# hyperconnect/TC-ResNet

Measured on AMD Instinct MI355X. Metric: utterances/sec (1 s@16 kHz) TCResNet8-1.0 forward, higher is better.
Workload: dtype f32; 1 GPU; TCResNet8-1.0 eval forward, waveform->softmax, batch 4096/GPU, 49x40 MFCC (40/20 ms, FFT 1024), 12 classes; global_batch=4096, parallelism=dp1 (utterance shards, no collective)

## Files before the change

include/tcresnet_hip.h:

```cpp
#ifndef TCRESNET_HIP_H
#define TCRESNET_HIP_H

#include <stddef.h>
#include <stdint.h>

#ifdef __cplusplus
extern "C" {
#endif

#define TCR_ABI_VERSION 3
#define TCR_HALO 4
#define TCR_MAX_BLOCKS 16

typedef enum tcr_status {
    TCR_OK = 0,
    TCR_ERR_ARG = -1,
    TCR_ERR_HIP = -2,
    TCR_ERR_WORKSPACE = -3
} tcr_status;

int tcr_abi_version(void);
const char* tcr_last_error(void);
static inline int tcr_padded_len(int t) { return t + 2 * TCR_HALO; }

// ... 230 lines not shown
                    float* logits, float* probs, float* smoothed, int32_t* top, float* score, int32_t* is_new, void* stream);

#define TCR_FAMILY_TCRESNET 0
#define TCR_FAMILY_DSCNN 1
#define TCR_FAMILY_G2D 2
typedef struct tcr_model_ref {
    int family;
    const void* handle;
    const float* params;
    const float* aux;
} tcr_model_ref;

size_t tcr_stream_state_bytes_m(const tcr_frontend_cfg* cfg, const tcr_model_ref* model, int n_streams, int k, const tcr_detect_cfg* det);
size_t tcr_stream_workspace_bytes_m(const tcr_frontend_cfg* cfg, const tcr_model_ref* model, int n_streams, int k);
int tcr_stream_init_m(const tcr_frontend_cfg* cfg, const void* plan_dev, const tcr_model_ref* model, int n_streams, int k,
                      const tcr_detect_cfg* det, void* state, void* workspace, size_t ws_bytes, void* stream);
int tcr_stream_step_m(const tcr_frontend_cfg* cfg, const void* plan_dev, const tcr_model_ref* model, int n_streams, int k,
                      const tcr_detect_cfg* det, const float* samples, const uint8_t* reset, void* state, void* workspace,
                      size_t ws_bytes, float* logits, float* probs, float* smoothed, int32_t* top, float* score, int32_t* is_new,
                      void* stream);
size_t tcr_scan_workspace_bytes_m(const tcr_frontend_cfg* cfg, const tcr_model_ref* model, int k, int max_windows);
int tcr_scan_m(const tcr_frontend_cfg* cfg, const void* plan_dev, const tcr_model_ref* model, int n_signals, int64_t n_samples, int k,
               const tcr_detect_cfg* det, const float* samples, void* workspace, size_t ws_bytes, float* logits, float* probs,
               float* smoothed, int32_t* top, float* score, int32_t* is_new, void* stream);
int tcr_stream_scan_m(const tcr_frontend_cfg* cfg, const void* plan_dev, const tcr_model_ref* model, int n_streams, int64_t n_samples,
                      int k, const tcr_detect_cfg* det, const float* samples, const uint8_t* reset, void* state, void* workspace,
                      size_t ws_bytes, float* logits, float* probs, float* smoothed, int32_t* top, float* score, int32_t* is_new,
                      void* stream);

int tcr_detect_sweep(int n_signals, int64_t steps, int num_classes, const int32_t* top, const float* score,
                     const int64_t* valid_steps, int32_t suppression_steps, int n_thresholds, const float* thresholds,
                     const int32_t* event_offsets, const int64_t* event_first, const int64_t* event_last,
                     const int32_t* event_label, int32_t* detections, int32_t* hits, int32_t* duplicates,
                     uint8_t* fired, void* stream);

typedef struct {
    int32_t up, down, taps;
    int32_t in_format;
    int32_t in_step;
} tcr_resample_cfg;
int tcr_resample(const tcr_resample_cfg* cfg, const float* table, int n_streams, const void* in, int64_t in_pitch, int64_t in_first,
                 int64_t n_in, int64_t out_first, int64_t n_out, float* out, int64_t out_pitch, void* stream);
int tcr_resample_span(const tcr_resample_cfg* cfg, int64_t out_first, int64_t n_out, int64_t* first, int64_t* n);

const char* tcr_kernel_name(int index);

enum { TCR_TUNE_CONV_PATH = 0,
       TCR_TUNE_FRONTEND = 1,
       TCR_TUNE_CONV_B = 2,
       TCR_TUNE_NET_FUSED = 3,
       TCR_TUNE_FUSED_GROUP = 4,
       TCR_TUNE_FUSED_WAVES = 5,
       TCR_TUNE_CONV_KSPLIT = 6,
       TCR_TUNE_WGRAD_STREAM = 7,
       TCR_TUNE_TRAIN_FWD = 8,
       TCR_TUNE_TRAIN_BWD = 9,
       TCR_TUNE_PHASE_CFG = 10,
       TCR_TUNE_BWD_BN_FUSED = 11,
       TCR_TUNE_BWD_MASK = 12,
       TCR_TUNE_FE_GRID = 13,
       TCR_TUNE_FUSED_GRID = 14,
       TCR_TUNE_DS_TRAIN = 15,
       TCR_TUNE_WGRAD_TILES = 16,
       TCR_TUNE_DOWN_DGRAD = 17,
       TCR_TUNE_BWD_LAZY_CFG = 18,
       TCR_TUNE_PHASE_STATIC = 19,
       TCR_TUNE_WGRAD_WAVES = 20,
       TCR_TUNE_WGRAD_LDS = 21,
       TCR_TUNE_LAZY_STAGE = 22,
       TCR_TUNE_FE_KERNEL = 23,
       TCR_TUNE_FE_STAGGER = 24,
       TCR_TUNE_PW_WGRAD = 25,
       TCR_TUNE_DEPLOY_F32 = 26,
       TCR_TUNE_NET_SMALL = 27,
       TCR_TUNE_PW_POS = 28,
       TCR_TUNE_BN_APPLY = 29,
       TCR_TUNE_DW_DGRAD = 30,
       TCR_TUNE_DW_WGRAD = 31,
       TCR_TUNE_DW_FWD = 32,
       TCR_TUNE_WGRAD_PIPE = 33,
       TCR_TUNE_COUNT = 34 };
int tcr_tune(int knob, int value);

void* tcr_internal_stream(int idx, void* caller_stream);

#ifdef __cplusplus
}
#endif
#endif
```

tc-resnet_amd/_lib.py:

```python
from __future__ import annotations

import ctypes as C
import os
from typing import Optional

HALO = 4
MAX_BLOCKS = 16
ABI_VERSION = 3
_HERE = os.path.dirname(os.path.abspath(__file__))
HIP_LIB_PATH = os.path.join(_HERE, "lib", "libtcresnet_hip.so")


class TcrError(RuntimeError):
    pass


class FrontendCfg(C.Structure):
    _fields_ = [("sample_rate", C.c_int32), ("n_samples", C.c_int32), ("win", C.c_int32), ("hop", C.c_int32),
                ("nfft", C.c_int32), ("n_frames", C.c_int32), ("n_mel", C.c_int32), ("n_coef", C.c_int32),
                ("lower_hz", C.c_float), ("upper_hz", C.c_float), ("method", C.c_int32)]


class TCResNetCfg(C.Structure):
    _fields_ = [("scope", C.c_char * 32), ("in_channels", C.c_int32), ("t_in", C.c_int32), ("num_classes", C.c_int32),
                ("n_blocks", C.c_int32), ("channels", C.c_int32 * (MAX_BLOCKS + 1)), ("bn_decay", C.c_float),
                ("bn_eps", C.c_float)]


class DSCNNCfg(C.Structure):
    _fields_ = [("h_in", C.c_int32), ("w_in", C.c_int32), ("num_classes", C.c_int32), ("depth", C.c_int32),
                ("n_separable", C.c_int32), ("conv1_kh", C.c_int32), ("conv1_kw", C.c_int32), ("conv1_sh", C.c_int32),
                ("conv1_sw", C.c_int32), ("ds1_sh", C.c_int32), ("ds1_sw", C.c_int32), ("bn_decay", C.c_float),
                ("bn_eps", C.c_float)]


class DetectCfg(C.Structure):
    _fields_ = [("average_steps", C.c_int32), ("min_count", C.c_int32), ("suppression_steps", C.c_int32), ("threshold", C.c_float)]


class ResampleCfg(C.Structure):
    _fields_ = [("up", C.c_int32), ("down", C.c_int32), ("taps", C.c_int32), ("in_format", C.c_int32), ("in_step", C.c_int32)]


FAMILY_TCRESNET, FAMILY_DSCNN, FAMILY_G2D = 0, 1, 2


class ModelRef(C.Structure):
    _fields_ = [("family", C.c_int), ("handle", C.c_void_p), ("params", C.c_void_p), ("aux", C.c_void_p)]


class TensorInfo(C.Structure):
    _fields_ = [("name", C.c_char * 96), ("kind", C.c_int32), ("arena", C.c_int32), ("offset", C.c_int64),
                ("size", C.c_int64), ("shape", C.c_int32 * 4), ("rank", C.c_int32)]


_P = C.c_void_p
_PROTOTYPES = {
    "tcr_abi_version": (C.c_int, []),
    "tcr_last_error": (C.c_char_p, []),
    "tcr_kernel_name": (C.c_char_p, [C.c_int]),
    "tcr_tune": (C.c_int, [C.c_int, C.c_int]),
    "tcr_internal_stream": (_P, [C.c_int, _P]),
    "tcr_frontend_resolve": (C.c_int, [C.POINTER(FrontendCfg)]),
    "tcr_frontend_plan_bytes": (C.c_size_t, [C.POINTER(FrontendCfg)]),
    "tcr_frontend_plan_init": (C.c_int, [C.POINTER(FrontendCfg), _P]),
    "tcr_frontend_plan_mel_matrix": (C.c_int, [C.POINTER(FrontendCfg), _P, _P]),
    "tcr_frontend_plan_dct_matrix": (C.c_int, [C.POINTER(FrontendCfg), _P, _P]),
    "tcr_frontend_fwd": (C.c_int, [C.POINTER(FrontendCfg), _P, _P, C.c_int, _P, _P]),
    "tcr_frontend_fwd_rounds": (C.c_int, [C.POINTER(FrontendCfg), _P, _P, C.c_int, _P, C.c_int, _P]),
    "tcr_features_to_planar": (C.c_int, [_P, C.c_int, C.c_int, C.c_int, _P, _P]),
    "tcr_features_from_planar": (C.c_int, [_P, C.c_int, C.c_int, C.c_int, _P, _P]),
    "tcr_tcresnet_create": (C.c_int, [C.POINTER(TCResNetCfg), C.POINTER(_P)]),
    "tcr_net_destroy": (None, [_P]),
    "tcr_net_param_floats": (C.c_int64, [_P]),
    "tcr_net_decay_floats": (C.c_int64, [_P]),
    "tcr_net_stat_floats": (C.c_int64, [_P]),
    "tcr_net_num_tensors": (C.c_int, [_P]),
    "tcr_net_tensor_info": (C.c_int, [_P, C.c_int, C.POINTER(TensorInfo)]),
    "tcr_net_out_frames": (C.c_int, [_P]),
    "tcr_net_feat_channels": (C.c_int, [_P]),
    "tcr_net_workspace_bytes": (C.c_size_t, [_P, C.c_int, C.c_int]),
    "tcr_net_forward_infer": (C.c_int, [_P, _P, _P, _P, C.c_int, _P, C.c_size_t, _P, _P, _P, _P]),
    "tcr_net_forward_train": (C.c_int, [_P, _P, _P, _P, _P, C.c_int, C.c_int, C.c_float, C.c_uint64, C.c_int64,
                                        C.c_float, _P, C.c_size_t, _P, _P, _P, _P]),
    "tcr_net_frozen_floats": (C.c_int64, [_P]),
    "tcr_net_fold_bn": (C.c_int, [_P, _P, _P, _P, _P]),
    "tcr_net_forward_frozen": (C.c_int, [_P, _P, _P, _P, C.c_int, _P, C.c_size_t, _P, _P, _P, _P]),
    "tcr_forward_waveform": (C.c_int, [C.POINTER(FrontendCfg), _P, _P, _P, _P, _P, C.c_int, _P, C.c_int, _P, _P, C.c_size_t, _P, _P, _P, _P]),
    "tcr_net_backward": (C.c_int, [_P, _P, _P, C.c_int, _P, C.c_size_t, _P, _P]),
    "tcr_net_num_stages": (C.c_int, [_P, C.c_int]),
    "tcr_net_stage_sums": (C.c_int, [_P, C.c_int, C.c_int, _P, C.c_int, C.POINTER(_P), C.POINTER(C.c_int64)]),
    "tcr_net_forward_train_stage": (C.c_int, [_P, _P, _P, _P, _P, C.c_int, C.c_int, C.c_float, C.c_uint64, C.c_int64,
                                              C.c_float, _P, C.c_size_t, _P, _P, _P, C.c_int, _P]),
    "tcr_net_backward_stage": (C.c_int, [_P, _P, _P, C.c_int, C.c_int, _P, C.c_size_t, _P, C.c_int, _P]),
    "tcr_net_num_levels": (C.c_int, [_P, C.c_int]),
    "tcr_net_level_sums": (C.c_int, [_P, C.c_int, C.c_int, _P, C.c_int, C.POINTER(_P), C.POINTER(C.c_int64)]),
    "tcr_net_forward_train_level": (C.c_int, [_P, _P, _P, _P, _P, C.c_int, C.c_int, C.c_float, C.c_uint64, C.c_int64,
                                              C.c_float, _P, C.c_size_t, _P, _P, _P, C.c_int, _P]),
    "tcr_net_backward_level": (C.c_int, [_P, _P, _P, C.c_int, C.c_int, _P, C.c_size_t, _P, C.c_int, _P]),
    "tcr_dscnn_create": (C.c_int, [C.POINTER(DSCNNCfg), C.POINTER(_P)]),
    "tcr_dscnn_destroy": (None, [_P]),
    "tcr_dscnn_param_floats": (C.c_int64, [_P]),
    "tcr_dscnn_stat_floats": (C.c_int64, [_P]),
    "tcr_dscnn_num_tensors": (C.c_int, [_P]),
    "tcr_dscnn_tensor_info": (C.c_int, [_P, C.c_int, C.POINTER(TensorInfo)]),
    "tcr_dscnn_workspace_bytes": (C.c_size_t, [_P, C.c_int]),
    "tcr_dscnn_forward_infer": (C.c_int, [_P, _P, _P, _P, C.c_int, _P, C.c_size_t, _P, _P, _P]),
    "tcr_augment_fwd": (C.c_int, [_P, _P, _P, _P, _P, _P, _P, C.c_int, C.c_int, _P, _P]),
    "tcr_dscnn_train_workspace_bytes": (C.c_size_t, [_P, C.c_int]),
    "tcr_dscnn_forward_train": (C.c_int, [_P, _P, _P, _P, _P, C.c_int, C.c_int, C.c_float, _P, C.c_size_t, _P, _P, _P, _P]),
    "tcr_dscnn_backward": (C.c_int, [_P, _P, _P, C.c_int, _P, C.c_size_t, _P, _P]),
    "tcr_dscnn_num_units": (C.c_int, [_P]),
    "tcr_dscnn_unit_output": (C.c_int, [_P, C.c_int, C.c_int, C.POINTER(C.c_int64), C.POINTER(C.c_int), C.POINTER(C.c_int), C.POINTER(C.c_int)]),
    "tcr_dscnn_materialize_unit": (C.c_int, [_P, C.c_int, C.c_int, _P, C.c_size_t, _P]),
    "tcr_dscnn_num_stages": (C.c_int, [_P]),
    "tcr_dscnn_stage_sums": (C.c_int, [_P, C.c_int, C.c_int, _P, C.c_int, C.POINTER(_P), C.POINTER(C.c_int64)]),
    "tcr_dscnn_forward_train_stage": (C.c_int, [_P, _P, _P, _P, _P, C.c_int, C.c_int, C.c_float, _P, C.c_size_t, _P, _P, _P, C.c_int, _P]),
    "tcr_dscnn_backward_stage": (C.c_int, [_P, _P, _P, C.c_int, C.c_int, _P, C.c_size_t, _P, C.c_int, _P]),
    "tcr_g2d_create": (C.c_int, [C.c_char_p, C.c_int, C.c_int, C.c_int, C.POINTER(_P)]),
    "tcr_g2d_destroy": (None, [_P]),
    "tcr_g2d_conv": (C.c_int, [_P, C.c_int, C.c_int, C.c_int, C.c_int, C.c_int, C.c_int, C.c_int, C.c_int, C.c_int, C.c_int, C.c_char_p,
                               C.c_char_p]),
    "tcr_g2d_batch_norm": (C.c_int, [_P, C.c_int, C.c_int, C.c_int, C.c_int, C.c_float, C.c_float, C.c_char_p]),
    "tcr_g2d_pool": (C.c_int, [_P, C.c_int, C.c_int, C.c_int, C.c_int, C.c_int, C.c_int, C.c_int]),
    "tcr_g2d_add": (C.c_int, [_P, C.c_int, C.c_int, C.c_int]),
    "tcr_g2d_dropout": (C.c_int, [_P, C.c_int, C.c_float]),
    "tcr_g2d_time_filter": (C.c_int, [_P, C.c_int, C.c_char_p]),
    "tcr_g2d_group_sum": (C.c_int, [_P, C.c_int, C.c_int, C.c_int, C.c_char_p]),
    "tcr_g2d_node_shape": (C.c_int, [_P, C.c_int, C.POINTER(C.c_int), C.POINTER(C.c_int), C.POINTER(C.c_int)]),
    "tcr_g2d_node_output": (C.c_int, [_P, C.c_int, C.c_int, C.c_int, C.POINTER(C.c_int64), C.POINTER(C.c_int64), C.POINTER(C.c_int)]),
    "tcr_g2d_finalize": (C.c_int, [_P, C.c_int]),
    "tcr_g2d_param_floats": (C.c_int64, [_P]),
    "tcr_g2d_decay_floats": (C.c_int64, [_P]),
    "tcr_g2d_stat_floats": (C.c_int64, [_P]),
    "tcr_g2d_num_tensors": (C.c_int, [_P]),
    "tcr_g2d_num_classes": (C.c_int, [_P]),
    "tcr_g2d_tensor_info": (C.c_int, [_P, C.c_int, C.POINTER(TensorInfo)]),
    "tcr_g2d_workspace_bytes": (C.c_size_t, [_P, C.c_int, C.c_int]),
    "tcr_g2d_input_from_features": (C.c_int, [_P, C.c_int, C.c_int, C.c_int, _P, _P]),
    "tcr_g2d_forward_infer": (C.c_int, [_P, _P, _P, _P, C.c_int, _P, C.c_size_t, _P, _P, _P]),
    "tcr_g2d_forward_train": (C.c_int, [_P, _P, _P, _P, _P, C.c_int, C.c_int, C.c_uint64, C.c_int64, C.c_float, _P, C.c_size_t, _P, _P, _P,
                                        _P]),
    "tcr_g2d_backward": (C.c_int, [_P, _P, _P, C.c_int, C.c_uint64, C.c_int64, _P, C.c_size_t, _P, _P]),
    "tcr_g2d_num_stages": (C.c_int, [_P]),
# ... 92 lines not shown
```

tc-resnet_amd/csrc/fused.hip:

```cpp
#include <cstdint>

#include "kernels.h"

namespace tcr {

typedef float f32x4 __attribute__((ext_vector_type(4)));

#ifndef TCR_FUSED_WHATIF
#define TCR_FUSED_WHATIF 0
#endif
#define TCR_WHATIF(bit) ((TCR_FUSED_WHATIF & (bit)) != 0)
#if TCR_FUSED_WHATIF & (16384 | 32768)
#define TCR_WHATIF_PRIO(bit, level) do { if (TCR_WHATIF(bit)) __builtin_amdgcn_s_setprio(level); } while (0)
#else
#define TCR_WHATIF_PRIO(bit, level) do { } while (0)
#endif
#if TCR_FUSED_WHATIF & 1
__device__ __forceinline__ f32x4 whatif_nomfma(float a, float b, f32x4 c) { c[0] += a; c[1] += b; return c; }
#define TCR_MFMA(A, B, C) whatif_nomfma((A), (B), (C))
#else
#define TCR_MFMA(A, B, C) __builtin_amdgcn_mfma_f32_16x16x4f32((A), (B), (C), 0, 0, 0)
#endif

template <int NW, int R>
// ... 299 lines not shown
#pragma unroll
            for (int reg = 0; reg < 4; ++reg) {
                const int co = min(m * 16 + q * 4 + reg, COUT - 1);
                rv[nt][reg] = res[gg[nt] * res_sz + co * TPO + kHalo + tt[nt]];
            }
    }
#pragma unroll
    for (int nt = 0; nt < NTJ; ++nt) {
        const bool pv = cc[nt] < npos;
        const f32x4 ac = acc[nt];
        const int base = gg[nt] * out_sz + kHalo + tt[nt];
#pragma unroll
        for (int reg = 0; reg < 4; ++reg) {
            const int co = m * 16 + q * 4 + reg;
            float v = fmaf(ac[reg], sc[reg], sh[reg]);
            if (HAS_RES) v = fmaxf(v + rv[nt][reg], 0.f);
            else v = fmaxf(v, lo);
            const bool ok = pv && (COUT % 16 == 0 || co < COUT) && !(TCR_WHATIF(32) && v != 12345.f);
            yout[ok ? base + co * TPO : dump - a.buf_off[L.out_buf]] = v;
        }
    }
}

template <int NW, int K, int S, int CIN, int COUT, int TIN, bool HAS_RES, int NTJ = 2, bool WLDS = false>
__device__ __forceinline__ void fused_layer_s(const FusedArgs& a, const FusedLayer& L, const float* __restrict__ xin, const int in_sz,
                                              float* lds, const int ng, const int wave, const int r_in, const int q_in,
                                              const int w_lds = 0) {
    const int oz = opaque_zero();
    const int r = r_in + oz, q = q_in + oz;
    constexpr int TOUT = (TIN + S - 1) / S;
    constexpr int NRT = (COUT + 15) / 16;
    constexpr int JP = 16 * NTJ;
    static_assert(CIN % 4 == 0, "channel quads");
    static_assert(NTJ == 1 || NTJ == 2 || NTJ == 4, "one, two or four 16-position tiles per job");
    float* yout = lds + a.buf_off[L.out_buf];
    const float* res = L.res_buf >= 0 ? lds + a.buf_off[L.res_buf] : nullptr;
    const int npos = ng * TOUT;
    const int ncp = (npos + JP - 1) / JP;
    const float* w = WLDS ? lds + w_lds : a.params + L.w_off;
    constexpr bool IL = S == 1;
    for (int job = wave; job < ncp * NRT; job += NW) {
        const int cp = job / NRT, m = job - cp * NRT;
        int cc[NTJ];
#pragma unroll
        for (int nt = 0; nt < NTJ; ++nt) cc[nt] = (IL && NTJ > 1) ? cp * JP + 32 * (nt >> 1) + 2 * r + (nt & 1) : cp * JP + 16 * nt + r;
        fused_job_s<K, S, CIN, COUT, TIN, HAS_RES, NTJ, WLDS>(a, L, xin, in_sz, yout, res, w, npos, m, cc, r, q);
    }
}

template <int NW, int K, int S, int CIN, int COUT, int TIN, bool HAS_RES, int AHEAD = 0>
__device__ __forceinline__ void fused_layer_u(const FusedArgs& a, const FusedLayer& L, const float* __restrict__ xin, const int in_sz,
                                              float* lds, const int ng, const int wave, const int r_in, const int q_in) {
    const int oz = opaque_zero();
    const int r = r_in + oz, q = q_in + oz;
    constexpr int TOUT = (TIN + S - 1) / S;
    constexpr int NRT = (COUT + 15) / 16;
    constexpr bool IL = S == 1;
    float* yout = lds + a.buf_off[L.out_buf];
    const float* res = L.res_buf >= 0 ? lds + a.buf_off[L.res_buf] : nullptr;
    const int npos = ng * TOUT;
    const int full = npos >> 5, rem = npos & 31;
    const int nt16 = IL ? 2 * full + (rem == 0 ? 0 : (rem <= 16 ? 1 : 2)) : (npos + 15) >> 4;
    const int il_end = (IL && rem > 0 && rem <= 16) ? 2 * full : nt16;
    const int U = NRT * nt16;
    const int per = U / NW, extra = U - per * NW;
    int u = wave * per + min(wave, extra);
    const int end = u + per + (wave < extra ? 1 : 0);
    const float* w = a.params + L.w_off;
    auto col = [&](int c) { return (IL && c < il_end) ? (c >> 1) * 32 + 2 * r + (c & 1) : (IL ? full * 32 + r : c * 16 + r); };
    while (u < end) {
        const int m = u / nt16, c = u - m * nt16;
        if (c + 1 < nt16 && u + 1 < end) {
            const int cc[2] = {col(c), col(c + 1)};
            fused_job_s<K, S, CIN, COUT, TIN, HAS_RES, 2, false, AHEAD>(a, L, xin, in_sz, yout, res, w, npos, m, cc, r, q);
            u += 2;
        } else {
            const int cc[1] = {col(c)};
            fused_job_s<K, S, CIN, COUT, TIN, HAS_RES, 1, false, AHEAD>(a, L, xin, in_sz, yout, res, w, npos, m, cc, r, q);
            u += 1;
        }
    }
}

template <int NW, int T0, bool WLDS = false>
__device__ __forceinline__ void fused_conv0_s(const FusedArgs& a, const FusedLayer& L, const float* __restrict__ xin, const int in_sz,
                                              float* lds, const int ng, const int wave, const int r_in, const int q_in,
                                              const int w_lds = 0) {
    const int oz = opaque_zero();
    const int r = r_in + oz, q = q_in + oz;
    constexpr int K = 3, CIN = 40, COUT = 16, C4 = CIN / 4;
    constexpr int TPI = T0 + 2 * kHalo, TPO = TPI, TOUT = T0, PADLO = 1;
    constexpr int WSTEP = 4 * COUT, XSTEP = 4 * TPI;
    float* yout = lds + a.buf_off[L.out_buf];
    const int out_sz = L.out_sz;
    const int npos = ng * TOUT;
    const int nct = (npos + 15) / 16;
    const float* w = WLDS ? lds + w_lds : a.params + L.w_off;
    const float* scale = a.ss + L.ss_off;
    const float* shift = scale + L.c_pad;
    for (int job = wave; job < nct; job += NW) {
        const int p0 = min(job * 16 + r, npos - 1);
        const int g0 = p0 / TOUT;
        const int t0 = p0 - g0 * TOUT;
        const float* wp = w + q * COUT + r;
        const float* x0 = xin + g0 * in_sz + q * TPI + t0 + kHalo - PADLO;
        float b0[C4][K], wf[K][C4];
#pragma unroll
        for (int c4 = 0; c4 < C4; ++c4)
#pragma unroll
            for (int j = 0; j < K; ++j) b0[c4][j] = x0[c4 * XSTEP + j];
#pragma unroll
        for (int j = 0; j < K; ++j)
#pragma unroll
            for (int c4 = 0; c4 < C4; ++c4) wf[j][c4] = wp[(j * C4 + c4) * WSTEP];
        float sc[4], sh[4];
#pragma unroll
        for (int reg = 0; reg < 4; ++reg) {
            sc[reg] = scale[q * 4 + reg];
            sh[reg] = shift[q * 4 + reg];
        }
        f32x4 acc0 = (f32x4){0.f, 0.f, 0.f, 0.f};
        TCR_WHATIF_PRIO(16384, 2);
#pragma unroll
        for (int j = 0; j < K; ++j)
#pragma unroll
            for (int c4 = 0; c4 < C4; ++c4) acc0 = TCR_MFMA(wf[j][c4], b0[c4][j], acc0);
        TCR_WHATIF_PRIO(16384, 0);
        const int dump = a.buf_off[2] + a.group * a.buf_sz[2] + (q * 16 + r) - a.buf_off[L.out_buf];
        const float lo = L.relu ? 0.f : -3.4e38f;
        const bool pv = job * 16 + r < npos;
        const int base = g0 * out_sz + kHalo + t0;
#pragma unroll
        for (int reg = 0; reg < 4; ++reg) {
            const float v = fmaxf(fmaf(acc0[reg], sc[reg], sh[reg]), lo);
            yout[pv ? base + (q * 4 + reg) * TPO : dump] = v;
        }
    }
}

template <int NT, int FC, int FT, int NCLS>
__device__ __forceinline__ void fused_head_s(const FusedArgs& a, float* lds, const int n0, const int ng, const int tid) {
    static_assert(FC % 4 == 0 && NCLS + 2 <= 16, "one 16-row MFMA tile holds the logits and the two range outputs");
    constexpr int TP = FT + 2 * kHalo;
    const float* fb = lds + a.buf_off[a.feat_buf];
    const int fsz = a.feat_sz;
    float* pooled = lds + a.buf_off[(a.feat_buf + 1) % 3];
    const int lane = tid & 63, r = lane & 15, q = lane >> 4;
    float af[FC / 4];
    if (tid < 64) {
        const int zero = opaque_zero();
#pragma unroll
        for (int s = 0; s < FC / 4; ++s) {
            const int c = 4 * s + q;
            const float* src = r < NCLS ? a.params + a.fc_off + c * NCLS + r : a.params + a.fc2_off + c * 2 + min(r - NCLS, 1);
            const float v = src[zero];
            af[s] = r < NCLS + 2 ? v : 0.f;
        }
    }
    for (int i = tid; i < ng * FC; i += NT) {
        const int g = i / FC, c = i - g * FC;
        const float* row = fb + g * fsz + c * TP + kHalo;
        float v[FT];
#pragma unroll
        for (int t = 0; t < FT; ++t) v[t] = row[t];
        float s = 0.f;
#pragma unroll
        for (int t = 0; t < FT; ++t) s += v[t];
        pooled[i] = s / (float)FT;
    }
    __syncthreads();
    if (tid < 64) {
        const int g = min(r, ng - 1);
        float bf[FC / 4];
#pragma unroll
        for (int s = 0; s < FC / 4; ++s) bf[s] = pooled[g * FC + 4 * s + q];
        f32x4 acc = (f32x4){0.f, 0.f, 0.f, 0.f};
#pragma unroll
        for (int s = 0; s < FC / 4; ++s) acc = __builtin_amdgcn_mfma_f32_16x16x4f32(af[s], bf[s], acc, 0, 0, 0);
        float mx = -3.0e38f;
#pragma unroll
        for (int reg = 0; reg < 4; ++reg) if (4 * q + reg < NCLS) mx = fmaxf(mx, acc[reg]);
        mx = fmaxf(mx, __shfl_xor(mx, 16));
        mx = fmaxf(mx, __shfl_xor(mx, 32));
        float e[4];
#pragma unroll
        for (int reg = 0; reg < 4; ++reg) e[reg] = expf(acc[reg] - mx);
        float se = 0.f;
#pragma unroll
        for (int row = 0; row < (NCLS + 3) / 4; ++row) {
            const float prev = __shfl(se, (row > 0 ? (row - 1) * 16 : 0) + r);
            float cur = row > 0 ? prev : 0.f;
#pragma unroll
            for (int reg = 0; reg < 4; ++reg) if (4 * row + reg < NCLS) cur += e[reg];
            if (q == row) se = cur;
        }
        se = __shfl(se, ((NCLS + 3) / 4 - 1) * 16 + r);
        if (r < ng) {
            const size_t n = (size_t)(n0 + r);
#pragma unroll
            for (int reg = 0; reg < 4; ++reg) {
                const int o = 4 * q + reg;
                if (o < NCLS) {
                    a.logits[n * NCLS + o] = acc[reg];
                    a.probs[n * NCLS + o] = e[reg] / se;
                } else if (o < NCLS + 2 && a.ranges) {
                    a.ranges[n * 2 + (o - NCLS)] = 1.0f / (1.0f + expf(-acc[reg]));
                }
            }
        }
    }
    __syncthreads();
}

template <int NT, int COUT, int TOUT>
__device__ __forceinline__ void fused_zero_halo(float* yout, const int out_sz, const int ng, const int tid_in) {
    constexpr int TPO = TOUT + 2 * kHalo;
    if (TCR_WHATIF(1024)) return;
    const int tid = tid_in + opaque_zero();
    for (int i = tid; i < ng * COUT * 2; i += NT) {
        const int row = i >> 1;
        const int g = row / COUT, co = row - g * COUT;
        float* p = yout + g * out_sz + co * TPO + ((i & 1) ? kHalo + TOUT : 0);
        p[0] = 0.f; p[1] = 0.f; p[2] = 0.f; p[3] = 0.f;
    }
}

template <int NT>
__device__ __forceinline__ void fused_head(const FusedArgs& a, float* lds, const int n0, const int ng, const int tid) {
    {
        const float* fb = lds + a.buf_off[a.feat_buf];
        const int fsz = a.feat_sz, tp = a.feat_t + 2 * kHalo;
        float* pooled = lds + a.buf_off[(a.feat_buf + 1) % 3];
        for (int i = tid; i < ng * a.feat_c; i += NT) {
            const int g = i / a.feat_c, c = i - g * a.feat_c;
            const float* row = fb + g * fsz + c * tp + kHalo;
            float s = 0.f;
            for (int t = 0; t < a.feat_t; ++t) s += row[t];
            pooled[i] = s / (float)a.feat_t;
        }
        __syncthreads();
        float* lg = pooled + a.group * a.feat_c;
        const int no = a.nc + 2;
        for (int i = tid; i < ng * no; i += NT) {
            const int g = i / no, o = i - g * no;
            const float* pv = pooled + g * a.feat_c;
            float s = 0.f;
            if (o < a.nc) {
                const float* wf = a.params + a.fc_off + o;
#pragma unroll 8
                for (int c = 0; c < a.feat_c; ++c) s = fmaf(pv[c], wf[(size_t)c * a.nc], s);
            } else {
                const float* wf = a.params + a.fc2_off + (o - a.nc);
#pragma unroll 8
                for (int c = 0; c < a.feat_c; ++c) s = fmaf(pv[c], wf[(size_t)c * 2], s);
            }
            lg[i] = s;
        }
        __syncthreads();
        for (int i = tid; i < ng * no; i += NT) {
            const int g = i / no, o = i - g * no;
            const float* z = lg + g * no;
            const size_t n = (size_t)(n0 + g);
            if (o < a.nc) {
                float mx = z[0];
                for (int k = 1; k < a.nc; ++k) mx = fmaxf(mx, z[k]);
                float se = 0.f;
                for (int k = 0; k < a.nc; ++k) se += expf(z[k] - mx);
                a.logits[n * a.nc + o] = z[o];
                a.probs[n * a.nc + o] = expf(z[o] - mx) / se;
            } else if (a.ranges) {
                a.ranges[n * 2 + (o - a.nc)] = 1.0f / (1.0f + expf(-z[o]));
            }
        }
        __syncthreads();
    }
}

#define TCR_WAVES_PER_SIMD_4 TCR_WAVES_PER_SIMD(4)
template <int NW, int K, int S, int CIN, int COUT, int TIN, int WD, bool HAS_RES, bool HALO = true, int NTJ = 2, bool WLDS = false>
__device__ __forceinline__ void fused_layer_sel(const FusedArgs& a, const FusedLayer& L, const float* __restrict__ xin, const int in_sz,
                                                float* lds, const int ng, const int wave, const int r, const int q,
                                                const int w_lds = 0) {
    if constexpr (WD < 0) fused_layer_t<NW, K, S, CIN, COUT, TIN>(a, L, xin, in_sz, lds, ng, wave, r, q);
    else {
        if constexpr (HALO) fused_zero_halo<NW * 64, COUT, (TIN + S - 1) / S>(lds + a.buf_off[L.out_buf], L.out_sz, ng, (int)threadIdx.x);
        if constexpr (NTJ == 0) fused_layer_u<NW, K, S, CIN, COUT, TIN, HAS_RES>(a, L, xin, in_sz, lds, ng, wave, r, q);
        else if constexpr (NTJ == 3) fused_layer_u<NW, K, S, CIN, COUT, TIN, HAS_RES, (CIN <= 32 ? 1 : 0)>(a, L, xin, in_sz, lds, ng, wave, r, q);
        else if constexpr (NTJ == 13) fused_layer_u<NW, K, S, CIN, COUT, TIN, HAS_RES, (CIN <= 48 ? 1 : 0)>(a, L, xin, in_sz, lds, ng, wave, r, q);
        else fused_layer_s<NW, K, S, CIN, COUT, TIN, HAS_RES, NTJ, WLDS>(a, L, xin, in_sz, lds, ng, wave, r, q, w_lds);
    }
}

template <int NW, int T0, int WD, int NTJ0 = 2>
__global__ __launch_bounds__(NW * 64) TCR_WAVES_PER_SIMD_4 void net_fused_tc8_kernel(const FusedArgs a) {
    constexpr int NT = NW * 64;
    constexpr int T1 = (T0 + 1) / 2, T2 = (T1 + 1) / 2;
    float* lds = reinterpret_cast<float*>(dyn_lds());
    const int tid = threadIdx.x;
    const int lane = tid & 63;
    const int wave = __builtin_amdgcn_readfirstlane(tid >> 6);
    const int r = lane & 15, q = lane >> 4;
    const int row = a.in_c * a.in_tp;
#if TCR_FUSED_WHATIF & 2048
    long long ts[14];
    int nts = 0;
#define TCR_TC8_BARRIER do { __syncthreads(); ts[nts++] = (long long)__builtin_readcyclecounter(); } while (0)
#elif TCR_FUSED_WHATIF & 8
#define TCR_TC8_BARRIER ((void)0)
#else
#define TCR_TC8_BARRIER __syncthreads()
#endif
#define TCR_TC8(LI, K_, S_, CI_, CO_, T_) fused_layer_sel<NW, K_, S_, CI_, CO_, T_, WD, (LI == 3 || LI == 6 || LI == 9), (K_ != 1 && LI != 9), ((LI >= 1 && LI <= 3 && NTJ0 == 4) ? 4 : (((NTJ0 == 0 || NTJ0 == 3) && K_ == 9) ? NTJ0 : 2))>(a, a.layer[LI], lds + a.buf_off[a.layer[LI].in_buf], a.layer[LI].in_sz, lds, ng, wave, r, q)
    for (int grp = blockIdx.x; grp < (TCR_WHATIF(512) ? 0 : a.n_groups); grp += gridDim.x) {
        const int n0 = grp * a.group;
        const int ng = min(a.group, a.batch - n0);
#if TCR_FUSED_WHATIF & 2048
        nts = 0;
        ts[nts++] = (long long)__builtin_readcyclecounter();
#endif
        if constexpr (WD < 0) fused_layer_sel<NW, 3, 1, 40, 16, T0, WD, false>(a, a.layer[0], a.feat + (size_t)n0 * row, row, lds, ng, wave, r, q);
        else if (!TCR_WHATIF(64)) {
            fused_zero_halo<NT, 16, T0>(lds + a.buf_off[a.layer[0].out_buf], a.layer[0].out_sz, ng, tid);
            fused_conv0_s<NW, T0>(a, a.layer[0], a.feat + (size_t)n0 * row, row, lds, ng, wave, r, q);
        }
        TCR_TC8_BARRIER;
        TCR_TC8(1, 1, 2, 16, 24, T0);
        TCR_TC8(2, 9, 2, 16, 24, T0);
        TCR_TC8_BARRIER;
        TCR_TC8(3, 9, 1, 24, 24, T1);
        TCR_TC8_BARRIER;
        TCR_TC8(4, 1, 2, 24, 32, T1);
        TCR_TC8(5, 9, 2, 24, 32, T1);
        TCR_TC8_BARRIER;
        TCR_TC8(6, 9, 1, 32, 32, T2);
        TCR_TC8_BARRIER;
        TCR_TC8(7, 1, 2, 32, 48, T2);
        TCR_TC8(8, 9, 2, 32, 48, T2);
        TCR_TC8_BARRIER;
        TCR_TC8(9, 9, 1, 48, 48, (T2 + 1) / 2);
        TCR_TC8_BARRIER;
        if constexpr (WD < 0) fused_head<NT>(a, lds, n0, ng, tid);
        else if (!TCR_WHATIF(16)) {
            if (a.nc == 12) fused_head_s<NT, 48, (T2 + 1) / 2, 12>(a, lds, n0, ng, tid);
            else fused_head<NT>(a, lds, n0, ng, tid);
        }
#if TCR_FUSED_WHATIF & 2048
        __syncthreads();
        ts[nts++] = (long long)__builtin_readcyclecounter();
        if (tid == 0)
            for (int i = 0; i + 1 < nts && i < 12; ++i) a.probs[(size_t)n0 * a.nc + i] = (float)(ts[i + 1] - ts[i]);
#endif
    }
#undef TCR_TC8
#undef TCR_TC8_BARRIER
}

template <int NW>
__device__ __forceinline__ void small_stage_weights(const float* __restrict__ src, int n_floats, float* dst, int wave, int lane) {
    for (int c0 = wave * 256; c0 < n_floats; c0 += NW * 256) {
        const int c = c0 + 4 * lane;
        if (c < n_floats) glds16(src + c, dst + c0);
    }
}

template <int NW, int T0>
__global__ __launch_bounds__(NW * 64) void net_small_tc8_kernel(const FusedArgs a, const int wa_off, const int wb_off) {
    constexpr int NT = NW * 64;
    constexpr int T1 = (T0 + 1) / 2, T2 = (T1 + 1) / 2, T3 = (T2 + 1) / 2;
    float* lds = reinterpret_cast<float*>(dyn_lds());
    const int tid = threadIdx.x;
    const int lane = tid & 63;
    const int wave = __builtin_amdgcn_readfirstlane(tid >> 6);
    const int r = lane & 15, q = lane >> 4;
    const int row = a.in_c * a.in_tp;
    float* WA = lds + wa_off;
    float* WB = lds + wb_off;
    constexpr int W0 = 3 * 40 * 16, WD0 = 16 * 24, W00 = 9 * 16 * 24, W01 = 9 * 24 * 24, WD1 = 24 * 32, W10 = 9 * 24 * 32, W11 = 9 * 32 * 32,
                  WD2 = 32 * 48, W20 = 9 * 32 * 48, W21 = 9 * 48 * 48;
#define TCR_SM_W(LI) (a.params + a.layer[LI].w_off)
#define TCR_SM(LI, K_, S_, CI_, CO_, T_, WP_) fused_layer_sel<NW, K_, S_, CI_, CO_, T_, 0, (LI == 3 || LI == 6 || LI == 9), (K_ != 1 && LI != 9), 1, true>(a, a.layer[LI], lds + a.buf_off[a.layer[LI].in_buf], a.layer[LI].in_sz, lds, 1, wave, r, q, WP_)
#if TCR_FUSED_WHATIF & 2048
    long long ts[16];
    int nts = 0;
#define TCR_SM_TS() ts[nts++] = (long long)__builtin_readcyclecounter()
#else
#define TCR_SM_TS() ((void)0)
#endif
    for (int n0 = blockIdx.x; n0 < a.batch; n0 += gridDim.x) {
        TCR_SM_TS();
        small_stage_weights<NW>(TCR_SM_W(0), W0, WA, wave, lane);
        small_stage_weights<NW>(TCR_SM_W(1), WD0, WB, wave, lane);
        small_stage_weights<NW>(TCR_SM_W(2), W00, WB + WD0, wave, lane);
        fused_zero_halo<NT, 16, T0>(lds + a.buf_off[a.layer[0].out_buf], a.layer[0].out_sz, 1, tid);
        wait_dma();
        __syncthreads();
        TCR_SM_TS();
        fused_conv0_s<NW, T0, true>(a, a.layer[0], a.feat + (size_t)n0 * row, row, lds, 1, wave, r, q, wa_off);
        __syncthreads();
        TCR_SM_TS();
        small_stage_weights<NW>(TCR_SM_W(3), W01, WA, wave, lane);
        TCR_SM(1, 1, 2, 16, 24, T0, wb_off);
        TCR_SM(2, 9, 2, 16, 24, T0, wb_off + WD0);
        wait_dma();
        __syncthreads();
        TCR_SM_TS();
        small_stage_weights<NW>(TCR_SM_W(4), WD1, WB, wave, lane);
        small_stage_weights<NW>(TCR_SM_W(5), W10, WB + WD1, wave, lane);
        TCR_SM(3, 9, 1, 24, 24, T1, wa_off);
        wait_dma();
        __syncthreads();
        TCR_SM_TS();
        small_stage_weights<NW>(TCR_SM_W(6), W11, WA, wave, lane);
        TCR_SM(4, 1, 2, 24, 32, T1, wb_off);
        TCR_SM(5, 9, 2, 24, 32, T1, wb_off + WD1);
        wait_dma();
        __syncthreads();
        TCR_SM_TS();
        small_stage_weights<NW>(TCR_SM_W(7), WD2, WB, wave, lane);
        small_stage_weights<NW>(TCR_SM_W(8), W20, WB + WD2, wave, lane);
        TCR_SM(6, 9, 1, 32, 32, T2, wa_off);
        wait_dma();
        __syncthreads();
        TCR_SM_TS();
        small_stage_weights<NW>(TCR_SM_W(9), W21, WA, wave, lane);
        TCR_SM(7, 1, 2, 32, 48, T2, wb_off);
        TCR_SM(8, 9, 2, 32, 48, T2, wb_off + WD2);
        wait_dma();
        __syncthreads();
        TCR_SM_TS();
        TCR_SM(9, 9, 1, 48, 48, T3, wa_off);
        __syncthreads();
        TCR_SM_TS();
        if (a.nc == 12) fused_head_s<NT, 48, T3, 12>(a, lds, n0, 1, tid);
        else fused_head<NT>(a, lds, n0, 1, tid);
#if TCR_FUSED_WHATIF & 2048
        __syncthreads();
// ... 222 lines not shown
                    a.logits[n * nc + o] = acc[reg];
                    a.probs[n * nc + o] = e[reg] / se;
                } else if (o < nc + 2 && a.ranges) {
                    a.ranges[n * 2 + (o - nc)] = 1.0f / (1.0f + expf(-acc[reg]));
                }
            }
        }
    }
    __syncthreads();
}

template <int NW, int R>
__global__ __launch_bounds__(NW * 64) void net_fused_kernel(const FusedArgs a) {
    constexpr int NT = NW * 64;
    float* lds = reinterpret_cast<float*>(dyn_lds());
    const int tid = threadIdx.x;
    const int lane = tid & 63;
    const int wave = __builtin_amdgcn_readfirstlane(tid >> 6);
    const int r = lane & 15, q = lane >> 4;

    for (int grp = blockIdx.x; grp < a.n_groups; grp += gridDim.x) {
        const int n0 = grp * a.group;
        const int ng = min(a.group, a.batch - n0);
        const int row = a.in_c * a.in_tp;
        if (!a.in_global) {
            const float4* src = reinterpret_cast<const float4*>(a.feat + (size_t)n0 * row);
            float4* dst = reinterpret_cast<float4*>(lds + a.buf_off[0]);
            const int nvec = ng * row / 4;
            for (int i = tid; i < nvec; i += NT) dst[i] = src[i];
            __syncthreads();
        }

        for (int li = 0; li < a.n_layers; ++li) {
            const FusedLayer L = a.layer[li];
            fused_zero_halo_g<NT>(lds + a.buf_off[L.out_buf], L.out_sz, ng, L.cout, L.tout, tid);
            if (li == 0 && a.in_global) {
                if (L.k == 3 && L.cin == 40 && L.stride == 1 && L.pad_lo == 1) fused_conv0_g<NW>(a, L, a.feat + (size_t)n0 * row, row, lds, ng, wave, r, q);
                else fused_layer<NW, R>(a, L, a.feat + (size_t)n0 * row, row, lds, ng, wave, r, q);
            } else {
                fused_layer<NW, R>(a, L, lds + a.buf_off[L.in_buf], L.in_sz, lds, ng, wave, r, q);
            }
            if (!L.no_barrier) __syncthreads();
        }

        if ((a.feat_c & 3) == 0 && a.nc + 2 <= 16) fused_head_g<NT>(a, lds, n0, ng, tid);
        else fused_head<NT>(a, lds, n0, ng, tid);
    }
}

static int launch_net_small(const FusedArgs& a0, hipStream_t s) {
    constexpr int kWA = 9 * 48 * 48, kWB = 32 * 48 + 9 * 32 * 48;
    FusedArgs a = a0;
    if (reinterpret_cast<uintptr_t>(a.params) % 16 != 0) return 1;
    for (int li = 0; li < a.n_layers; ++li)
        if (a.layer[li].w_off % 4 != 0) return 1;
    const int act = a.buf_off[2] + a.buf_sz[2];
    const int wa_off = (act + 64 + 63) / 64 * 64, wb_off = wa_off + kWA + 64;
    const size_t lds = ((size_t)wb_off + kWB + 64) * sizeof(float);
    if (lds > 160 * 1024) return 1;
    static bool configured = false;
    if (!configured) {
        if (hipFuncSetAttribute(reinterpret_cast<const void*>(net_small_tc8_kernel<8, 49>), hipFuncAttributeMaxDynamicSharedMemorySize, 160 * 1024) != hipSuccess) {
            (void)hipGetLastError();
            return 1;
        }
        configured = true;
    }
    hipLaunchKernelGGL((net_small_tc8_kernel<8, 49>), dim3(a.batch), dim3(512), lds, s, a, wa_off, wb_off);
    return check_launch("net_small_tc8_kernel");
}

int launch_net_fused(const FusedArgs& a, size_t lds_bytes, int grid, int waves, int ring, hipStream_t s) {
    void (*kern)(const FusedArgs) = nullptr;
    const int tc8 = tune_get(TCR_TUNE_NET_FUSED) == 3 ? 0 : fused_tc8_frames(a);
    if (tc8 == 49 && a.group == 1 && a.batch <= kSmallBatchMax && a.nc + 2 <= 16 && tune_get(TCR_TUNE_NET_FUSED) == 0 && tune_get(TCR_TUNE_NET_SMALL) == 0 &&
        tune_get(TCR_TUNE_FUSED_WAVES) == 0) {
        const int rc = launch_net_small(a, s);
        if (rc != 1) return rc;
    }
    const bool r2 = tune_get(TCR_TUNE_NET_FUSED) == 4;
    const bool j2 = tune_get(TCR_TUNE_NET_FUSED) == 8;
    const bool ju = tune_get(TCR_TUNE_NET_FUSED) == 9;
    const bool j4 = tune_get(TCR_TUNE_NET_FUSED) == 5;
#define TCR_FS(NW_, T_) if (tc8 == T_ && waves == NW_) kern = r2 ? net_fused_tc8_kernel<NW_, T_, -1> : (j4 ? net_fused_tc8_kernel<NW_, T_, 0, 4> : (ju ? net_fused_tc8_kernel<NW_, T_, 0, 0> : (j2 ? net_fused_tc8_kernel<NW_, T_, 0, 2> : net_fused_tc8_kernel<NW_, T_, 0, 3>)));
    TCR_FS(4, 49) TCR_FS(8, 49) TCR_FS(16, 49) TCR_FS(4, 98) TCR_FS(8, 98) TCR_FS(16, 98)
#undef TCR_FS
    const int tc14 = (kern || tune_get(TCR_TUNE_NET_FUSED) == 3 || tune_get(TCR_TUNE_NET_FUSED) == 4) ? 0 : fused_tc14w_frames(a);
#define TCR_F14(NW_, T_) if (tc14 == T_ && waves == NW_) kern = ju ? net_fused_tc14w_kernel<NW_, T_, 0> : (j2 ? net_fused_tc14w_kernel<NW_, T_, 2> : net_fused_tc14w_kernel<NW_, T_, 13>);
    TCR_F14(8, 49) TCR_F14(16, 49) TCR_F14(8, 98) TCR_F14(16, 98)
#undef TCR_F14
    if (kern) ring = 0;
#define TCR_FK(NW_, R_) if (!kern && waves == NW_ && ring == R_) kern = net_fused_kernel<NW_, R_>;
    TCR_FK(4, 4) TCR_FK(4, 8) TCR_FK(4, 16) TCR_FK(8, 4) TCR_FK(8, 8) TCR_FK(8, 16) TCR_FK(16, 4) TCR_FK(16, 8) TCR_FK(16, 16)
#undef TCR_FK
    if (!kern) { set_error("fused kernel: no instantiation for %d waves / ring %d", waves, ring); return TCR_ERR_ARG; }
    if (lds_bytes > 64 * 1024) {
        if (hipFuncSetAttribute(reinterpret_cast<const void*>(kern), hipFuncAttributeMaxDynamicSharedMemorySize, (int)lds_bytes) != hipSuccess) {
            (void)hipGetLastError();
            return 1;
        }
    }
    hipLaunchKernelGGL(kern, dim3(grid), dim3(waves * 64), lds_bytes, s, a);
    return check_launch("net_fused_kernel");
}

}
```

tc-resnet_amd/csrc/kernels.h:

```cpp
#pragma once
#include "tcr_common.h"

namespace tcr {

enum ConvEpilogue { EPI_RAW = 0, EPI_AFFINE = 1 };

struct ConvArgs {
    const float* x;
    const float* w;
    float* y;
    const float* scale;
    const float* shift;
    const float* res;
    int npos;
    int cin, cout;
    int tpi, tout, tpo;
    int xoff;
    int relu;
    int ostride, ooff;
    const float* add;
    const float* add_mask;
    int add_bcast;
};

// ... 60 lines not shown
int launch_conv_dgrad_mfma(int k, int stride, int pad_lo, const float* w, float* wt, const float* dy, float* dx, const float* add,
                           const float* add_mask, int add_bcast, int batch, int cin, int cout, int tin, int tout, hipStream_t s,
                           bool wt_ready = false, unsigned add_phases = ~0u);
unsigned conv_dgrad_phases(int k, int stride, int pad_lo, int tin);
bool conv_dgrad_mfma_covers(int k, int stride, int cout);
int launch_conv_mfma_with_down(const ConvArgs& a, const float* w_down, float* y_down, const float* scale_down,
                               const float* shift_down, int pad_lo, int epi, hipStream_t s);
size_t wgrad_partial_floats(int k, int cin, int cout, int batch, bool fine = false);
int wgrad_chunks(int batch);
int wgrad_chunks_for(int batch, bool fine);
int launch_wgrad_reduce(const float* partial, float* dw, int nchunk, int k, int cin, int cout, int cin_pad, int cout_pad,
                        int cout_all, int co_base, hipStream_t s);
int launch_conv_wgrad(int k, int stride, int pad_lo, const float* x, const float* dy, float* dw, float* scratch,
                      int batch, int cin, int cout, int tpi, int tout, int tpo, hipStream_t s,
                      const float* x_scale = nullptr, const float* x_shift = nullptr, bool x_slack = false);
constexpr int kMultiMax = 64;
struct WgradReduceEntry {
    const float* partial;
    float* dw;
    int nchunk, k, cin, cout, cin_pad, cout_pad;
};
struct WgradReduceMulti {
    int n;
    WgradReduceEntry e[kMultiMax];
};
bool conv_wgrad_deferrable(int k, int cin, int cout);
bool conv_wgrad_fly_covers(int k, int stride, bool x_slack);
struct WgradFly;
int launch_conv_wgrad_partial(int k, int stride, int pad_lo, const float* x, const float* dy, float* scratch, int batch, int cin, int cout,
                              int tpi, int tout, int tpo, WgradReduceEntry* entry, hipStream_t s, bool fine = false, bool x_slack = false,
                              const WgradFly* fly = nullptr);
WgradReduceEntry conv_wgrad_entry(int k, int cin, int cout, int batch, const float* scratch, float* dw, bool fine = false);
int launch_wgrad_reduce_multi(const WgradReduceMulti& m, hipStream_t s);
struct DgradWeightsEntry {
    const float* w;
    float* wt;
    int k, cin, cout, stride, pad_lo;
};
struct DgradWeightsMulti {
    int n;
    DgradWeightsEntry e[kMultiMax];
};
int launch_dgrad_weights_multi(const DgradWeightsMulti& m, hipStream_t s);
struct BwdPrologueArgs {
    const float* dlogits;
    const float* wfc;
    const float* dscale;
    float* dpool;
    int batch, c, nc;
    float* zero;
    int64_t zero_n;
};
int launch_bwd_prologue(const BwdPrologueArgs& h, const DgradWeightsMulti& m, hipStream_t s);

constexpr int kFusedMaxLayers = 32;

struct FusedLayer {
    int k, stride, cin, cout, tin, tout, pad_lo, relu;
    int in_buf, out_buf, res_buf;
    int w_off, ss_off, c_pad;
    int no_barrier;
    int in_sz, out_sz, res_sz;
};

struct FusedArgs {
    const float* params;
    const float* ss;
    const float* feat;
    float* logits;
    float* probs;
    float* ranges;
    int batch, group, n_groups, n_layers;
    int buf_off[3];
    int buf_sz[3];
    int in_c, in_tp;
    int feat_buf;
    int feat_c, feat_t, nc;
    int feat_sz;
    int fc_off, fc2_off;
    int in_global;
    FusedLayer layer[kFusedMaxLayers];
};

constexpr int kSmallBatchMax = 64;
int launch_net_fused(const FusedArgs& a, size_t lds_bytes, int grid, int waves, int ring, hipStream_t s);

constexpr int kPhaseMaxRows = 1024;
struct PhaseSrc {
    int kind;
    const float* a;
    const float* ss_a;
    int c_pad_a;
    int s_kind;
    const float* s;
    const float* ss_s;
    int c_pad_s;
    float* out_x;
    float* out_s;
    int c, t;
};
struct PhaseLayer {
    int k, stride, cin, cout, tin, tout, pad_lo;
    int w_off;
    float* raw;
    float* partial;
};
struct TrainPhaseArgs {
    const float* params;
    PhaseSrc src;
    int n_layers;
    PhaseLayer layer[2];
    int batch;
    float* pool_sum = nullptr;
    int group, n_groups, in_sz, cstat, stat_off, nw;
    int vec_stage = 0, tab_off = 0;
};
int launch_train_phase(TrainPhaseArgs a, int* rows_out, hipStream_t s);
int train_phase_rows(const TrainPhaseArgs& a);

struct BwdSrc {
    int kind;
    const float* da;
    int bcast;
    const float* m1;
    const float* m2;
    const float* raw;
    const float* mean;
    const float* k1;
    const float* k2;
    const float* k3;
    float* out_dy;
    int c, t;
};
struct BwdLayer {
    int src;
    int k, stride, pad_lo;
    int cin, tin;
    int cout, tout;
    const float* wt;
};
struct BwdStat {
    int on;
    const float* m1;
    const float* m2;
    const float* raw;
    const float* mean;
    const float* invstd;
    float* partial;
};
struct TrainBwdPhaseArgs {
    BwdSrc src[2];
    int n_layers;
    BwdLayer layer[2];
    int out_c, out_t;
    float* out_dx;
    const float* add;
    const float* add_mask;
    int add_bcast;
    BwdStat stat[2];
    int batch;
    int group, n_groups, src_sz[2], out_sz, src_off[2], out_off, cstat, stat_off, tpc, nw;
};
int launch_train_bwd_phase(TrainBwdPhaseArgs a, int* rows_out, hipStream_t s);
int train_bwd_phase_rows(const TrainBwdPhaseArgs& a);

struct LazySrc {
// ... 243 lines not shown
```

Before: 18.88 million utterances/s.

## Keep layer-3 conv weights register-resident and prefetch them before the barrier

Adds a register-resident variant for the stride-1 24->24 k=9 layer in the TC-ResNet8 fused kernel. Each wave owns one 16-row output tile and a fixed, rotated run of column tiles, and loads its weight fragment into registers once, issued before the preceding barrier so the fetch overlaps the wait. This removes repeated per-job weight reloads. The variant becomes the default for 49-frame inputs, at the cost of higher register pressure that may reduce occupancy. A host-callable helper exposing the wave-to-tile dealing, plus a small head-loader tweak, are also added.

```diff
diff --git a/include/tcresnet_hip.h b/include/tcresnet_hip.h
--- a/include/tcresnet_hip.h
+++ b/include/tcresnet_hip.h
@@ -336,6 +336,8 @@
        TCR_TUNE_COUNT = 34 };
 int tcr_tune(int knob, int value);
 
+int tcr_fused_deal_run(int nrt, int nt16, int nw, int wave, int* out3);
+
 void* tcr_internal_stream(int idx, void* caller_stream);
 
 #ifdef __cplusplus
diff --git a/tc-resnet_amd/_lib.py b/tc-resnet_amd/_lib.py
--- a/tc-resnet_amd/_lib.py
+++ b/tc-resnet_amd/_lib.py
@@ -60,6 +60,7 @@
     "tcr_last_error": (C.c_char_p, []),
     "tcr_kernel_name": (C.c_char_p, [C.c_int]),
     "tcr_tune": (C.c_int, [C.c_int, C.c_int]),
+    "tcr_fused_deal_run": (C.c_int, [C.c_int, C.c_int, C.c_int, C.c_int, C.POINTER(C.c_int)]),
     "tcr_internal_stream": (_P, [C.c_int, _P]),
     "tcr_frontend_resolve": (C.c_int, [C.POINTER(FrontendCfg)]),
     "tcr_frontend_plan_bytes": (C.c_size_t, [C.POINTER(FrontendCfg)]),
diff --git a/tc-resnet_amd/csrc/fused.hip b/tc-resnet_amd/csrc/fused.hip
--- a/tc-resnet_amd/csrc/fused.hip
+++ b/tc-resnet_amd/csrc/fused.hip
@@ -405,6 +405,101 @@
     }
 }
 
+template <int NW, int K, int CIN, int COUT>
+__device__ __forceinline__ void fused_resident_request(const FusedArgs& a, const FusedLayer& L, const int wave, const int r_in, const int q_in,
+                                                       float (&ws)[K * (CIN / 4)]) {
+    constexpr int NRT = (COUT + 15) / 16, C4 = CIN / 4, WSTEP = 4 * COUT;
+    static_assert(NW % NRT == 0, "the waves split evenly over the row tiles");
+    const int oz = opaque_zero();
+    const int r = r_in + oz, q = q_in + oz;
+    const int m = wave / (NW / NRT);
+    const buf_rsrc wr = make_rsrc(a.params + L.w_off);
+    const unsigned wl = (unsigned)(q * COUT + min(m * 16 + r, COUT - 1)) * 4u;
+#pragma unroll
+    for (int i = 0; i < K * C4; ++i) ws[i] = buf_load_f32(wr, wl, (unsigned)(i * WSTEP) * 4u);
+}
+
+template <int NW, int K, int S, int CIN, int COUT, int TIN, bool HAS_RES>
+__device__ __forceinline__ void fused_layer_r(const FusedArgs& a, const FusedLayer& L, const float* __restrict__ xin, const int in_sz,
+                                              float* lds, const int ng, const int wave, const int r_in, const int q_in,
+                                              const float (&ws)[K * (CIN / 4)]) {
+    const int oz = opaque_zero();
+    const int r = r_in + oz, q = q_in + oz;
+    constexpr int TOUT = (TIN + S - 1) / S;
+    constexpr int NRT = (COUT + 15) / 16;
+    constexpr bool IL = S == 1;
+    constexpr int PADT = ((TOUT - 1) * S + K - TIN) > 0 ? ((TOUT - 1) * S + K - TIN) : 0;
+    constexpr int PADLO = PADT / 2;
+    constexpr int TPI = TIN + 2 * kHalo, TPO = TOUT + 2 * kHalo;
+    constexpr int C4 = CIN / 4, XSTEP = 4 * TPI;
+    float* yout = lds + a.buf_off[L.out_buf];
+    const float* res = L.res_buf >= 0 ? lds + a.buf_off[L.res_buf] : nullptr;
+    const int out_sz = L.out_sz;
+    const int res_sz = L.res_sz;
+    const int npos = ng * TOUT;
+    const int full = npos >> 5, rem = npos & 31;
+    const int nt16 = IL ? 2 * full + (rem == 0 ? 0 : (rem <= 16 ? 1 : 2)) : (npos + 15) >> 4;
+    const int il_end = (IL && rem > 0 && rem <= 16) ? 2 * full : nt16;
+    const FusedRun run = fused_deal_run(NRT, nt16, NW, wave);
+    const int m = run.m;
+    const float* scale = a.ss + L.ss_off;
+    const float* shift = scale + L.c_pad;
+    float sc[4], sh[4];
+#pragma unroll
+    for (int reg = 0; reg < 4; ++reg) {
+        const int co = min(m * 16 + q * 4 + reg, COUT - 1);
+        sc[reg] = scale[co];
+        sh[reg] = shift[co];
+    }
+    auto place = [&](const int c, const int rr, int& g, int& t) {
+        const int cc = (IL && c < il_end) ? (c >> 1) * 32 + 2 * rr + (c & 1) : (IL ? full * 32 + rr : c * 16 + rr);
+        const int p = min(cc, npos - 1);
+        g = p / TOUT;
+        t = p - g * TOUT;
+        return cc < npos;
+    };
+    for (int c = run.c0; c < run.c1; ++c) {
+        int g, t;
+        place(c, r, g, t);
+        const float* xp = xin + g * in_sz + q * TPI + t * S + kHalo - PADLO;
+        f32x4 acc = (f32x4){0.f, 0.f, 0.f, 0.f};
+        float b[C4];
+#pragma unroll
+        for (int c4 = 0; c4 < C4; ++c4) b[c4] = xp[c4 * XSTEP];
+#pragma unroll
+        for (int j = 0; j < K; ++j) {
+#pragma unroll
+            for (int c4 = 0; c4 < C4; ++c4) {
+                acc = TCR_MFMA(ws[j * C4 + c4], b[c4], acc);
+                if (j + 1 < K) b[c4] = xp[c4 * XSTEP + (TCR_WHATIF(4) ? 0 : j + 1)];
+            }
+        }
+        const int oe = opaque_zero_after(acc[0]);
+        const int re = r_in + oe, qe = q_in + oe;
+        const bool pv = place(c, re, g, t);
+        const int dump = a.buf_off[2] + a.group * a.buf_sz[2] + (qe * 16 + re) - a.buf_off[L.out_buf];
+        const float lo = L.relu ? 0.f : -3.4e38f;
+        float rv[4];
+        if (HAS_RES) {
+#pragma unroll
+            for (int reg = 0; reg < 4; ++reg) {
+                const int co = min(m * 16 + qe * 4 + reg, COUT - 1);
+                rv[reg] = res[g * res_sz + co * TPO + kHalo + t];
+            }
+        }
+        const int base = g * out_sz + kHalo + t;
+#pragma unroll
+        for (int reg = 0; reg < 4; ++reg) {
+            const int co = m * 16 + qe * 4 + reg;
+            float v = fmaf(acc[reg], sc[reg], sh[reg]);
+            if (HAS_RES) v = fmaxf(v + rv[reg], 0.f);
+            else v = fmaxf(v, lo);
+            const bool ok = pv && (COUT % 16 == 0 || co < COUT) && !(TCR_WHATIF(32) && v != 12345.f);
+            yout[ok ? base + co * TPO : dump] = v;
+        }
+    }
+}
+
 template <int NW, int T0, bool WLDS = false>
 __device__ __forceinline__ void fused_conv0_s(const FusedArgs& a, const FusedLayer& L, const float* __restrict__ xin, const int in_sz,
                                               float* lds, const int ng, const int wave, const int r_in, const int q_in,
@@ -472,12 +567,13 @@
     float af[FC / 4];
     if (tid < 64) {
         const int zero = opaque_zero();
+        const int rz = r + zero, qz = q + zero;
 #pragma unroll
         for (int s = 0; s < FC / 4; ++s) {
-            const int c = 4 * s + q;
-            const float* src = r < NCLS ? a.params + a.fc_off + c * NCLS + r : a.params + a.fc2_off + c * 2 + min(r - NCLS, 1);
-            const float v = src[zero];
-            af[s] = r < NCLS + 2 ? v : 0.f;
+            const int c = 4 * s + qz;
+            const float* src = rz < NCLS ? a.params + a.fc_off + c * NCLS + rz : a.params + a.fc2_off + c * 2 + min(rz - NCLS, 1);
+            const float v = src[0];
+            af[s] = rz < NCLS + 2 ? v : 0.f;
         }
     }
     for (int i = tid; i < ng * FC; i += NT) {
@@ -633,7 +729,12 @@
 #else
 #define TCR_TC8_BARRIER __syncthreads()
 #endif
-#define TCR_TC8(LI, K_, S_, CI_, CO_, T_) fused_layer_sel<NW, K_, S_, CI_, CO_, T_, WD, (LI == 3 || LI == 6 || LI == 9), (K_ != 1 && LI != 9), ((LI >= 1 && LI <= 3 && NTJ0 == 4) ? 4 : (((NTJ0 == 0 || NTJ0 == 3) && K_ == 9) ? NTJ0 : 2))>(a, a.layer[LI], lds + a.buf_off[a.layer[LI].in_buf], a.layer[LI].in_sz, lds, ng, wave, r, q)
+    constexpr bool RES = WD >= 0 && NTJ0 == 6;
+    constexpr int NTJU = RES ? 3 : NTJ0;
+#define TCR_TC8(LI, K_, S_, CI_, CO_, T_) fused_layer_sel<NW, K_, S_, CI_, CO_, T_, WD, (LI == 3 || LI == 6 || LI == 9), (K_ != 1 && LI != 9), ((LI >= 1 && LI <= 3 && NTJU == 4) ? 4 : (((NTJU == 0 || NTJU == 3) && K_ == 9) ? NTJU : 2))>(a, a.layer[LI], lds + a.buf_off[a.layer[LI].in_buf], a.layer[LI].in_sz, lds, ng, wave, r, q)
+#define TCR_TC8_R(LI, S_, CI_, T_, WS_) do { \
+        fused_zero_halo<NT, 24, (T_ + S_ - 1) / S_>(lds + a.buf_off[a.layer[LI].out_buf], a.layer[LI].out_sz, ng, tid); \
+        fused_layer_r<NW, 9, S_, CI_, 24, T_, (LI == 3)>(a, a.layer[LI], lds + a.buf_off[a.layer[LI].in_buf], a.layer[LI].in_sz, lds, ng, wave, r, q, WS_); } while (0)
     for (int grp = blockIdx.x; grp < (TCR_WHATIF(512) ? 0 : a.n_groups); grp += gridDim.x) {
         const int n0 = grp * a.group;
         const int ng = min(a.group, a.batch - n0);
@@ -646,12 +747,23 @@
             fused_zero_halo<NT, 16, T0>(lds + a.buf_off[a.layer[0].out_buf], a.layer[0].out_sz, ng, tid);
             fused_conv0_s<NW, T0>(a, a.layer[0], a.feat + (size_t)n0 * row, row, lds, ng, wave, r, q);
         }
+        if constexpr (RES) {
+            float ws3[9 * 6];
+            TCR_TC8_BARRIER;
+            TCR_TC8(1, 1, 2, 16, 24, T0);
+            TCR_TC8(2, 9, 2, 16, 24, T0);
+            fused_resident_request<NW, 9, 24, 24>(a, a.layer[3], wave, r, q, ws3);
+            TCR_TC8_BARRIER;
+            TCR_TC8_R(3, 1, 24, T1, ws3);
+            TCR_TC8_BARRIER;
+        } else {
         TCR_TC8_BARRIER;
         TCR_TC8(1, 1, 2, 16, 24, T0);
         TCR_TC8(2, 9, 2, 16, 24, T0);
         TCR_TC8_BARRIER;
         TCR_TC8(3, 9, 1, 24, 24, T1);
         TCR_TC8_BARRIER;
+        }
         TCR_TC8(4, 1, 2, 24, 32, T1);
         TCR_TC8(5, 9, 2, 24, 32, T1);
         TCR_TC8_BARRIER;
@@ -675,6 +787,7 @@
 #endif
     }
 #undef TCR_TC8
+#undef TCR_TC8_R
 #undef TCR_TC8_BARRIER
 }
 
@@ -1063,7 +1176,9 @@
     const bool j2 = tune_get(TCR_TUNE_NET_FUSED) == 8;
     const bool ju = tune_get(TCR_TUNE_NET_FUSED) == 9;
     const bool j4 = tune_get(TCR_TUNE_NET_FUSED) == 5;
-#define TCR_FS(NW_, T_) if (tc8 == T_ && waves == NW_) kern = r2 ? net_fused_tc8_kernel<NW_, T_, -1> : (j4 ? net_fused_tc8_kernel<NW_, T_, 0, 4> : (ju ? net_fused_tc8_kernel<NW_, T_, 0, 0> : (j2 ? net_fused_tc8_kernel<NW_, T_, 0, 2> : net_fused_tc8_kernel<NW_, T_, 0, 3>)));
+    const bool jl = tune_get(TCR_TUNE_NET_FUSED) == 10;
+    const bool jr = tune_get(TCR_TUNE_NET_FUSED) == 11;
+#define TCR_FS(NW_, T_) if (tc8 == T_ && waves == NW_) kern = r2 ? net_fused_tc8_kernel<NW_, T_, -1> : (j4 ? net_fused_tc8_kernel<NW_, T_, 0, 4> : (ju ? net_fused_tc8_kernel<NW_, T_, 0, 0> : (j2 ? net_fused_tc8_kernel<NW_, T_, 0, 2> : ((jr || (T_ == 49 && !jl)) ? net_fused_tc8_kernel<NW_, T_, 0, 6> : net_fused_tc8_kernel<NW_, T_, 0, 3>))));
     TCR_FS(4, 49) TCR_FS(8, 49) TCR_FS(16, 49) TCR_FS(4, 98) TCR_FS(8, 98) TCR_FS(16, 98)
 #undef TCR_FS
     const int tc14 = (kern || tune_get(TCR_TUNE_NET_FUSED) == 3 || tune_get(TCR_TUNE_NET_FUSED) == 4) ? 0 : fused_tc14w_frames(a);
@@ -1086,3 +1201,13 @@
 }
 
 }
+
+extern "C" int tcr_fused_deal_run(int nrt, int nt16, int nw, int wave, int* out3) {
+    if (!out3 || nrt < 1 || nt16 < 0 || nw < nrt || nw % nrt != 0 || wave < 0 || wave >= nw) {
+        tcr::set_error("tcr_fused_deal_run: bad arguments (%d row tiles, %d column tiles, wave %d of %d)", nrt, nt16, wave, nw);
+        return TCR_ERR_ARG;
+    }
+    const tcr::FusedRun run = tcr::fused_deal_run(nrt, nt16, nw, wave);
+    out3[0] = run.m; out3[1] = run.c0; out3[2] = run.c1;
+    return TCR_OK;
+}
diff --git a/tc-resnet_amd/csrc/kernels.h b/tc-resnet_amd/csrc/kernels.h
--- a/tc-resnet_amd/csrc/kernels.h
+++ b/tc-resnet_amd/csrc/kernels.h
@@ -166,6 +166,16 @@
     FusedLayer layer[kFusedMaxLayers];
 };
 
+struct FusedRun { int m, c0, c1; };
+__host__ __device__ inline FusedRun fused_deal_run(const int nrt, const int nt16, const int nw, const int wave) {
+    const int wpt = nw / nrt;
+    const int m = wave / wpt, l = wave - m * wpt;
+    const int per = nt16 / wpt, extra = nt16 - per * wpt;
+    const int rank = (l + wpt - (m * extra) % wpt) % wpt;
+    const int c0 = rank * per + (rank < extra ? rank : extra);
+    return FusedRun{m, c0, c0 + per + (rank < extra ? 1 : 0)};
+}
+
 constexpr int kSmallBatchMax = 64;
 int launch_net_fused(const FusedArgs& a, size_t lds_bytes, int grid, int waves, int ring, hipStream_t s);
 
```

Measured after the change: 19.17 million utterances/s, median of 6. 1.02x the previous value.
